# bhansconnect/alphazero-pybind11

Hardware: AMD Instinct MI355X
Metric: self-play games/sec (whole node), Connect4 @ 800 MCTS sims (higher is better)
Workload: dtype bf16

## Files before the change

### alphazero-pybind11_amd/csrc/engine_kernels.h

```cpp
#pragma once
#include <hip/hip_runtime.h>
#include <stdint.h>

#include "dev_games.h"
#include "dev_rng.h"
#include "engine_types.h"

namespace azmi {

constexpr float kNoiseAlphaRatio = 10.83f;

__device__ __forceinline__ uint32_t seat_param(const uint32_t (&a)[4], uint32_t seat) {
  return seat == 0 ? a[0] : seat == 1 ? a[1] : seat == 2 ? a[2] : a[3];
}

__device__ __forceinline__ uint32_t gum_plan(uint32_t m, uint32_t n, uint32_t want, uint32_t& num_c_out, uint32_t& v_per_out) {
  num_c_out = 0; v_per_out = 0;
  if (m <= 1) { if (want == 0) { num_c_out = 1; v_per_out = n; } return 1; }
  uint32_t log2m = 0;
  for (uint32_t v = m - 1; v > 0; v >>= 1) ++log2m;
  if (log2m == 0) log2m = 1;
  const uint32_t d0 = n / (log2m * m);
  const uint32_t base_v = d0 > 1u ? d0 : 1u;
  uint32_t sims_used = 0, num_c = m, count = 0;
// ... 118 lines not shown
  }
  __device__ __forceinline__ size_t tree_base(uint32_t seat) const {
    return (static_cast<size_t>(slot) * P + seat) * ep.cap;
  }
  __device__ __forceinline__ uint32_t tree_id(uint32_t seat) const { return slot * P + seat; }
  __device__ __forceinline__ void raise(uint32_t bit) const {
    if (lane == 0) { atomicOr(&ar.ctl->overflow, bit); ar.ctl->stop = 1; }
  }
  __device__ __forceinline__ void sync_lanes() const { __builtin_amdgcn_fence(__ATOMIC_ACQ_REL, "workgroup"); }
  __device__ __forceinline__ void trace(uint64_t tag) const {
    if (slot != ep.trace_slot || lane != 0) return;
    const uint64_t val = (tag & 0xFF) >= 100 ? wall_clock64() : rng.state;
    if (ar.ctl->rounds < ep.trace_after) return;
    const uint64_t n = ar.trace[0];
    if (n + 1 < ep.trace_cap) { ar.trace[2 * (n + 1)] = tag; ar.trace[2 * (n + 1) + 1] = val; ar.trace[0] = n + 1; }
  }

  __device__ __forceinline__ void load() {
    rng.state = ar.rng[slot];
    coin.state = ar.coin[slot];
    flags = ar.flags[slot];
    const uint64_t w0 = ar.gs_words[0 * ep.S + slot], w1 = ar.gs_words[1 * ep.S + slot],
                   w2 = ar.gs_words[2 * ep.S + slot];
    gs.bb[0] = w0; gs.bb[1] = w1;
    gs.turn = static_cast<uint32_t>(w2); gs.player = static_cast<uint32_t>(w2 >> 32);
#pragma unroll
    for (int p = 0; p < P; ++p) {
      const uint32_t t = slot * P + p;
      t_root[p] = ar.root[t]; t_bump[p] = ar.bump[t]; t_depth[p] = ar.depth[t]; t_tld[p] = ar.tld[t];
    }
    cur = ar.cur[slot]; plen = ar.plen[slot]; ph_rows = ar.ph_count[slot];
    perm = ar.perm[slot];
#pragma unroll
    for (int p = 0; p < P; ++p) {
      const uint32_t* rec = ar.seat_tab + (static_cast<size_t>(perm) * P + p) * kSeatWords;
      sv_w0[p] = rec[0]; sv_w1[p] = rec[1]; sv_eps[p] = __uint_as_float(rec[2]); sv_rt[p] = __uint_as_float(rec[3]);
    }
  }
  __device__ __forceinline__ void store(uint8_t sstate) const {
    if (lane != 0) return;
    ar.rng[slot] = rng.state;
    ar.coin[slot] = coin.state;
    ar.flags[slot] = flags;
    ar.sstate[slot] = sstate;
    ar.gs_words[0 * ep.S + slot] = gs.bb[0];
    ar.gs_words[1 * ep.S + slot] = gs.bb[1];
    ar.gs_words[2 * ep.S + slot] = static_cast<uint64_t>(gs.turn) | (static_cast<uint64_t>(gs.player) << 32);
#pragma unroll
    for (int p = 0; p < P; ++p) {
      const uint32_t t = slot * P + p;
      ar.root[t] = t_root[p]; ar.bump[t] = t_bump[p]; ar.depth[t] = t_depth[p]; ar.tld[t] = t_tld[p];
    }
    ar.cur[slot] = cur; ar.plen[slot] = plen; ar.ph_count[slot] = ph_rows;
  }

  __device__ __forceinline__ void reset_tree(uint32_t seat) {
#pragma unroll
    for (int p = 0; p < P; ++p)
      if (static_cast<uint32_t>(p) == seat) { t_root[p] = 0; t_bump[p] = 1; t_depth[p] = 0; t_tld[p] = 0; }
    const size_t tb = tree_base(seat);
    if (lane == 0) { ar.nodes[tb].n = 0; ar.nodes[tb].q = 0; ar.nodes[tb].pr = 0; ar.nodes[tb].d = 0; ar.nodes[tb].v = 0; ar.nodes[tb].meta = 0; }
    if (ep.gumbel_on) set_gumbel_num_sims(seat, 0);
  }

  enum { kGumTarget = 0, kGumInit = 1, kGumNSurv = 2, kGumPhase = 3, kGumSims = 4, kGumMEff = 5, kGumRemain = 6 };
  __device__ __forceinline__ uint32_t* gum_state(uint32_t seat) const { return ar.gum_state + static_cast<size_t>(tree_id(seat)) * 8; }
  __device__ __forceinline__ float* gum_g(uint32_t seat) const { return ar.gum_g + static_cast<size_t>(tree_id(seat)) * ep.gum_stride; }
  __device__ __forceinline__ uint16_t* gum_surv(uint32_t seat) const { return ar.gum_surv + static_cast<size_t>(tree_id(seat)) * kGumMaxM; }

  __device__ __forceinline__ void reset_gumbel_state(uint32_t seat) const {
    if (lane != 0) return;
    uint32_t* st = gum_state(seat);
    st[kGumInit] = 0; st[kGumNSurv] = 0; st[kGumPhase] = 0; st[kGumSims] = 0; st[kGumMEff] = 0; st[kGumRemain] = 0;
  }
  __device__ __forceinline__ void set_gumbel_num_sims(uint32_t seat, uint32_t n) const {
    if (lane == 0) gum_state(seat)[kGumTarget] = n;
    reset_gumbel_state(seat);
  }
  __device__ __forceinline__ void set_gumbel_target() const {
    if (!ep.gumbel_on) return;
    const uint32_t cp = gs.player;
    const uint32_t target = (flags & kFlagCapped) ? (ep.fast_gumbel ? seat_cap_visits(cp) : 0u) : seat_visits(cp);
    set_gumbel_num_sims(cp, target);
  }
  __device__ __forceinline__ float gumbel01() {
    return 0.0f - 1.0f * az_logf(-az_logf(1.0f - canonical01(rng)));
  }
  __device__ __forceinline__ uint32_t group_max(uint32_t x) const {
    for (int off = 1; off < G; off <<= 1) x = max(x, __shfl_xor(x, off, G));
    return x;
  }
  __device__ __forceinline__ void init_gumbel_state(uint32_t seat, uint32_t k, float p_l) {
    if (k == 0) return;
    uint32_t* st = gum_state(seat);
    const uint32_t target = st[kGumTarget], depth = AZMI_SEL(t_depth, seat);
    const uint32_t remaining = depth < target ? target - depth : 0u;
    if (remaining == 0) return;
    const uint32_t gm = seat_gumbel_m(seat);
    uint32_t m_eff = gm < k ? gm : k;
    m_eff = m_eff < remaining ? m_eff : remaining;
    m_eff = m_eff > 1u ? m_eff : 1u;
    float g_l = 0.0f;
    for (uint32_t i = 0; i < k; ++i) { const float gi = gumbel01(); if (lane == i) g_l = gi; }
    const float score_l = g_l + az_logf(p_l + 1e-20f);
    uint32_t rank_l = 0;
    for (uint32_t j = 0; j < k; ++j) {
// ... 818 lines not shown
              if (b < np) dp[b] = t1;
              if (c < np) dp[c] = t2;
              if (d < np) dp[d] = t3;
            }
            float* dv = ar.h_v + dst0 * (P + 1);
            for (uint32_t e = lane; e < nr * (P + 1); e += G) dv[e] = (e % (P + 1) == term - 1) ? 1.0f : 0.0f;
            for (uint32_t r = lane; r < nr; r += G) {
              const uint32_t* pm = ar.ph_meta + (src0 + sr + r) * 2;
              uint32_t* hm = ar.h_meta + (dst0 + r) * 4;
              hm[0] = slot; hm[1] = game_idx; hm[2] = pm[1]; hm[3] = pm[0];
            }
          }
        }
      } else {
        raise(2u);
      }
    }
    ph_rows = 0;
    if (lane == 0) {
      atomicAdd(&ar.a_scores[static_cast<size_t>(slot) * (P + 1) + (term - 1)], 1.0f);
      if (resigned) atomicAdd(&ar.a_resign[static_cast<size_t>(slot) * (P + 1) + (term - 1)], 1.0f);
      atomicAdd(&ar.a_perm_scores[(static_cast<size_t>(slot) * ep.num_perms + perm) * (P + 1) + (term - 1)], 1.0f);
      atomicAdd(&ar.a_perm_games[static_cast<size_t>(slot) * ep.num_perms + perm], 1u);
      double gd[5]; uint32_t gc[3];
#pragma unroll
      for (int j = 0; j < 5; ++j) gd[j] = ar.g_dsum[j * S + slot];
#pragma unroll
      for (int j = 0; j < 3; ++j) gc[j] = ar.g_cnt[j * S + slot];
      atomicAdd(reinterpret_cast<unsigned long long*>(&ar.a_len[slot]), static_cast<unsigned long long>(gs.turn));
#pragma unroll
      for (int j = 0; j < 5; ++j) { atomicAdd(&ar.a_dsum[j * S + slot], gd[j]); ar.g_dsum[j * S + slot] = 0.0; }
#pragma unroll
      for (int j = 0; j < 3; ++j) { atomicAdd(reinterpret_cast<unsigned long long*>(&ar.a_cnt[j * S + slot]), static_cast<unsigned long long>(gc[j])); ar.g_cnt[j * S + slot] = 0; }
      atomicAdd(&ar.slot_games[slot], 1u);
      const uint32_t pos = atomicAdd(&ar.ctl->ended_count, 1u);
      ar.ended_list[pos] = slot;
    }
  }

  __device__ __forceinline__ void emit_leaf(const typename GM::State& leaf, uint64_t key) const {
    float* row = ar.canon + static_cast<size_t>(slot) * GM::CANON;
    for (uint32_t e = lane; e < static_cast<uint32_t>(GM::CANON); e += G) row[e] = GM::canonical_at(leaf, e);
    if (lane == 0) {
      ar.leaf_key[slot] = key;
      if (ar.leaf_pos) {
        ar.leaf_pos[0 * static_cast<size_t>(ep.S) + slot] = leaf.bb[0];
        ar.leaf_pos[1 * static_cast<size_t>(ep.S) + slot] = leaf.bb[1];
        ar.leaf_pos[2 * static_cast<size_t>(ep.S) + slot] = leaf.player;
      }
    }
  }
  struct NoEarly { __device__ __forceinline__ bool operator()(int, float&, float&) const { return false; } };
  struct NoAfter { __device__ __forceinline__ void operator()(float, float) const {} };
  template <class F = NoPreload, class E = NoEarly, class A = NoAfter>
  __device__ __forceinline__ bool cache_lookup(uint64_t key, uint32_t group, float& hit_pi, float& hit_v, F&& before_loads = F(), E&& early = E(),
                                               A&& after_hit = A()) const {
    uint32_t sh;
    const CacheView cache = ep.num_groups == 1 ? ar.cache : ar.caches[group];
    const int cslot = wave_shard_find<G>(cache, key, lane, &sh, before_loads);
    if (lane == 0) {
      unsigned long long* st = cache.stats + static_cast<size_t>(sh) * 4;
      if (cslot < 0) {
        atomicAdd(&st[1], 1ULL);
      } else {
        atomicAdd(&st[0], 1ULL);
        uint32_t* f = cache.freq + static_cast<size_t>(sh) * kWaveCap + cslot;
        atomicAdd(f, 1u);
        atomicMin(f, 3u);
      }
    }
    static_assert(M <= G, "one lane per policy entry");
    bool have = early(cslot, hit_pi, hit_v);
    if (!have) {
      if (cslot < 0) return false;
      const float* sp = cache.policy + (static_cast<size_t>(sh) * cache.cap + cslot) * M;
      const float* sv = cache.value + (static_cast<size_t>(sh) * cache.cap + cslot) * (P + 1);
      hit_pi = lane < static_cast<uint32_t>(M) ? sp[lane] : 0.0f;
      hit_v = lane <= static_cast<uint32_t>(P) ? sv[lane] : 0.0f;
      after_hit(hit_pi, hit_v);
    }
    if (lane < static_cast<uint32_t>(M)) ar.pi[static_cast<size_t>(slot) * M + lane] = hit_pi;
    if (lane <= static_cast<uint32_t>(P)) ar.v[static_cast<size_t>(slot) * (P + 1) + lane] = hit_v;
    return true;
  }
};

template <class GM, bool kPlayout = false, bool kMover = false>
__device__ __forceinline__ uint32_t round_slot(const EngineParams& ep, const EngineArrays& ar, const uint32_t slot, const uint32_t lane) {
  constexpr int G = GM::GROUP;
  constexpr int P = GM::P;
  if (slot >= ep.S) return 0xFFu;
  if (ar.ctl->stop) return 0xFFu;
  const uint8_t st = ar.sstate[slot];
  if (st == kSlotDone || st == kSlotEnded) { if (ep.cache_on && lane == 0) ar.cache_keys[slot] = 0; return 0xFFu; }
  if constexpr (!kMover) {
    if (st == kSlotQueued) {
      if (lane == 0) {
        const uint32_t group = ar.leaf_group[slot];
        if (ep.cache_on) ar.cache_keys[slot] = cache_key(ar.leaf_key[slot]);
        ar.eval_list[static_cast<size_t>(group) * ep.S + atomicAdd(&ar.ctl->eval_count[group], 1u)] = slot;
        ar.sstate[slot] = kSlotWaitEval;
      }
      return kSlotWaitEval;
    }
  }
  SlotCtx<GM> c(ep, ar, slot, lane);
  c.trace(100);
  c.load();
  if constexpr (kMover) c.flags &= ~kFlagListed;
  c.trace(101);
  uint32_t inline_sims = 0, insert_key_set = 0;
  PathRegs prec;
  bool need_process = (st == kSlotWaitEval);
  if (!need_process) {
    c.start_game();
    c.draw_capped();
    c.set_gumbel_target();
    if (ep.gumbel_on && st == kSlotRestart && !ep.tree_reuse) c.set_gumbel_num_sims(c.gs.player, 0);
  }
  bool have_regs = false;
  float reg_pi = 0.0f, reg_v = 0.0f;
  for (;;) {
    if (need_process) {
      const uint32_t cp = c.gs.player;
      const bool noise = c.seat_eps(cp) > 0 && !(c.flags & kFlagCapped);
      c.process_result(cp, (c.flags & kFlagLeafNeedsNet) != 0, noise, have_regs, reg_pi, reg_v);
      have_regs = false;
      c.trace(102);
      const uint32_t goal = (c.flags & kFlagCapped) ? c.seat_cap_visits(cp) : c.seat_visits(cp);
      if (AZMI_SEL(c.t_depth, cp) >= goal) {
        if (c.make_move(cp)) { if (ep.cache_on && lane == 0) ar.cache_keys[slot] = 0; c.store(kSlotEnded); c.trace(107); return kSlotEnded; }
        c.trace(103);
      }
    }
    const uint32_t cp = c.gs.player;
// ... 310 lines not shown
```

### alphazero-pybind11_amd/csrc/pipe_tree_kernels.h

```cpp
#pragma once
#include "engine_kernels.h"
#include "pipe_types.h"

namespace azmi {

__device__ __forceinline__ unsigned long long g_ld(const unsigned long long* p) { return __hip_atomic_load(p, __ATOMIC_RELAXED, __HIP_MEMORY_SCOPE_AGENT); }
__device__ __forceinline__ uint32_t g_ld(const uint32_t* p) { return __hip_atomic_load(p, __ATOMIC_RELAXED, __HIP_MEMORY_SCOPE_AGENT); }
__device__ __forceinline__ void g_st(unsigned long long* p, unsigned long long v) { __hip_atomic_store(p, v, __ATOMIC_RELAXED, __HIP_MEMORY_SCOPE_AGENT); }
__device__ __forceinline__ void g_st(uint32_t* p, uint32_t v) { __hip_atomic_store(p, v, __ATOMIC_RELAXED, __HIP_MEMORY_SCOPE_AGENT); }


enum : uint32_t { kGrpIdle = 0, kGrpReady = 1, kGrpWait = 2, kGrpPush = 3 };
constexpr uint64_t kFreezeTicks = 200000ull;
__device__ __forceinline__ void pipe_freeze_credit(PipeCtl* pc, uint64_t now, uint64_t& t_last, uint64_t& t_start, bool leader) {
  const uint64_t gap = now - t_last;
  if (gap > kFreezeTicks) {
    t_start += gap;
    if (leader) { atomicAdd(&pc->freezes, 1ull); atomicMax(&pc->freeze_max, static_cast<unsigned long long>(gap)); }
  }
  t_last = now;
}
constexpr uint64_t kMask48 = (1ull << 48) - 1;
constexpr uint32_t kNoSlot = 0xFFFFFFFFu;

// ... 80 lines not shown
    const unsigned long long em = __ballot(on && lane == 0 && res_state == kSlotEnded);
    const unsigned long long dm = __ballot(on && lane == 0 && (res_state == kSlotDone || res_state == 0xFFu));
    const unsigned long long om = __ballot(on && lane == 0);
    const unsigned long long sm = __ballot(on && lane == 0 && was_sim != 0u);
    if (wlane == 0) {
      if (em) atomicAdd(&pe->ended, static_cast<uint32_t>(__popcll(em)));
      if (dm) atomicAdd(&pe->dead, static_cast<uint32_t>(__popcll(dm)));
      if (sm) atomicAdd(&pe->sims, static_cast<unsigned long long>(__popcll(sm)));
      atomicAdd(&pe->moved, static_cast<uint32_t>(__popcll(om)));
    }
  }
  return res_state;
}

#ifndef AZMI_TREE_MINB
#define AZMI_TREE_MINB 2
#endif
template <class GM, int NT, bool PROF, bool TWO = false, bool GUM = false>
__global__ __launch_bounds__(NT, AZMI_TREE_MINB) void k_pipe_tree(PipeKernArgs ka) {
  constexpr int G = GM::GROUP;
  constexpr int P = GM::P;
  static_assert(P == 2 && G == 8 && GM::M == 7, "written for Connect4's 8-lane groups");
  const EngineParams& ep = ka.ep;
  const EngineArrays& ar = ka.ar;
  const PipeArrays& pa = ka.pa;
  const uint32_t wlane = threadIdx.x & 63u, grp = wlane >> 3, lane0 = wlane & 7u;
  uint64_t t_start = wall_clock64(), t_last = t_start;
  PipeCtl* const pc = pa.ctl;
  PipeEpoch* const pe = pa.ep;
  PipeWg* const wc = pa.wg + blockIdx.x;
  const uint32_t rmask = (1u << pa.rshift) - 1u;
  unsigned long long* const myring = pa.rring + (static_cast<size_t>(blockIdx.x) << pa.rshift);
  if (threadIdx.x == 0) {
    unsigned long long t0 = atomicCAS(&pe->t0, 0ull, static_cast<unsigned long long>(t_start));
    if (t0 == 0ull) t0 = t_start;
    atomicMax(&pe->tree_late, static_cast<uint32_t>(t_start > t0 ? t_start - t0 : 0ull));
    const uint32_t before = atomicAdd(&pe->tree_arrived, 1u);
    asm volatile("s_waitcnt vmcnt(0)" :: "v"(before) : "memory");
  }
  __syncthreads();
  if (pa.census_hold != 0u) {
    const unsigned long long t0 = g_ld(&pe->t0);
    if (threadIdx.x == 0 && t_start > t0 && t_start - t0 >= pa.census_hold) atomicAdd(&pe->tree_late_n, 1u);
    while (wall_clock64() < t0 + pa.census_hold) __builtin_amdgcn_s_sleep(32);
    return;
  }
  bool go = g_ld(&ar.ctl->stop) == 0 && g_ld(&pc->err) == 0 && g_ld(&pe->stop) == 0;
  __shared__ uint32_t s_head;
  if (threadIdx.x == 0) s_head = wc->rhead;
  __syncthreads();
  uint64_t pf_pass = 0, pf_idle = 0, pf_n = 0, pf_act = 0, pf_polls = 0, pf_io = 0, pf_lvls = 0, pf_mv = 0;
  uint64_t pf_ph[5] = {0, 0, 0, 0, 0};
  SlotCtx<GM> c(ep, ar, 0u, lane0);

  while (go) {
    const uint64_t pf_t0 = PROF ? wall_clock64() : 0;
    uint32_t lane = lane0;
    asm volatile("" : "+v"(lane));
    c.lane = lane;
    uint32_t my_slot = kNoSlot, tok_seq = 0, tok_move = 0, n_tok = 0, empty_polls = 0, ctl_word = 0;
    uint64_t t_seen = 0;
    bool fresh_pass = true;
    for (;;) {
      const uint32_t h = __builtin_amdgcn_readfirstlane(*const_cast<volatile uint32_t*>(&s_head));
      unsigned long long tok = 0;
      bool here = false;
      if (lane == 0) {
        const uint32_t pos = h + grp;
        tok = g_ld(myring + (pos & rmask));
        here = (tok >> 48) == pipe_lap_tag_r(pos, pa.rshift);
      }
      if ((empty_polls & 3u) == 0u) {
        ctl_word = 0;
        if (wlane == 7) ctl_word = g_ld(&pe->stop) | g_ld(&pc->err) | g_ld(&ar.ctl->stop);
        else if (wlane == 15) ctl_word = g_ld(&pe->sims) >= pa.quota ? 1u : 0u;
        else if (wlane == 23) ctl_word = g_ld(&pe->ended);
        else if (wlane == 31) ctl_word = g_ld(&pe->dead);
      }
      uint32_t stop_seen = __builtin_amdgcn_readlane(ctl_word, 7) | __builtin_amdgcn_readlane(ctl_word, 15);
      {
        const uint32_t w = __builtin_amdgcn_readlane(ctl_word, 23), d = __builtin_amdgcn_readlane(ctl_word, 31);
        const uint32_t with_game = ep.S > d ? ep.S - d : 0u;
        const uint32_t thr = max(1u, static_cast<uint32_t>((static_cast<unsigned long long>(with_game) * pa.idle_num) >> 10));
        if (w >= thr || w + d >= ep.S) stop_seen = 1u;
      }
      const uint64_t now = wall_clock64();
      if (fresh_pass) { t_last = now; fresh_pass = false; }
      else pipe_freeze_credit(pc, now, t_last, t_start, wlane == 0);
      if (now - t_start > pa.soft_ticks) stop_seen = 1u;
      if (now - t_start > pa.cap_ticks) {
        if (wlane == 0) { atomicOr(&pc->err, static_cast<uint32_t>(kPipeErrTimeout)); pc->dbg[16] = __builtin_amdgcn_readlane(ctl_word, 23); pc->dbg[17] = __builtin_amdgcn_readlane(ctl_word, 31); }
        stop_seen = 1u;
      }
      if (stop_seen) {
        if (wlane == 0) g_st(&pe->stop, 1u);
        go = false;
        break;
      }
      if constexpr (PROF) pf_polls += 1;
      const unsigned long long hm = __ballot(here);
      uint32_t k = 0;
      while (k < kTreeWindow && ((hm >> (8 * k)) & 1ull)) ++k;
      if (k == 0u) { ++empty_polls; __builtin_amdgcn_s_sleep(16); continue; }
      if (k < kTreeWindow && pa.take_wait != 0u) {
        if (t_seen == 0) t_seen = now;
        if (now - t_seen <= pa.take_wait) { __builtin_amdgcn_s_sleep(2); continue; }
      }
      uint32_t won = 0;
      if (wlane == 0) won = atomicCAS(&s_head, h, h + k) == h ? 1u : 0u;
      if (__builtin_amdgcn_readfirstlane(won) == 0u) continue;
      n_tok = k;
      {
        const uint32_t sl = static_cast<uint32_t>(__shfl(static_cast<uint32_t>(tok & 0xFFFFull), static_cast<int>(grp * 8), 64));
        const uint32_t sq = static_cast<uint32_t>(__shfl(static_cast<uint32_t>((tok >> 16) & 0xFFFFFFFFull), static_cast<int>(grp * 8), 64));
        if (grp < k) { my_slot = sl & static_cast<uint32_t>(kTokSlotMask); tok_move = (sl >> 15) & 1u; tok_seq = sq; }
      }
      break;
    }
    if (!go) break;
    const uint64_t pf_t1 = PROF ? wall_clock64() : 0;
    if constexpr (PROF) { pf_idle += pf_t1 - pf_t0; pf_n += 1; pf_act += n_tok; }

    if (__ballot(tok_move != 0u) != 0ull) {
      const PipeKernArgs* const kargs = reinterpret_cast<const PipeKernArgs*>(reinterpret_cast<uintptr_t>(__builtin_amdgcn_kernarg_segment_ptr()));
      const uint32_t rs = pipe_move_groups<GM>(kargs->ep, kargs->ar, kargs->pa, tok_move != 0u ? my_slot : kNoSlot);
      asm volatile("s_waitcnt vmcnt(0)" ::: "memory");
      if (tok_move != 0u) { if (rs == kSlotWaitEval) tok_seq = 0u; else my_slot = kNoSlot; }
      if constexpr (PROF) pf_mv += wall_clock64() - pf_t1;
    }

    const uint32_t slot = my_slot != kNoSlot ? my_slot : 0u;
    c.slot = slot;
    uint32_t st = kGrpIdle;
    uint8_t final_state = kSlotWaitEval;
    uint32_t cp = 0, root = 0, goal = 0, seq = 0, mg = 0, gum_active = 0, gum_full = 0;
    bool gum_defer = false;
    size_t tb = 0;
    float fpu_root = 0.0f;
    uint32_t* const path = ar.path + static_cast<size_t>(slot) * ep.max_depth;
    unsigned long long* const res = pa.res + static_cast<size_t>(slot) * kResStride;
    float reg_pi = 0.0f, reg_v = 0.0f;
    uint32_t root_n = 0; float root_v = 0.0f; uint64_t root_meta = 0;
    uint32_t lv_node = 0, lv_n = 0, lv_pp = 0;
    float lv_q = 0.0f, lv_d = 0.0f, lv_v = 0.0f;
    uint64_t lf_meta = 0;
    uint32_t lf_mv = 0, lf_c0 = 0, lf_k = 0, lf_term = 0, lf_player = 0;
    bool fw = false;
    uint32_t fw_node = 0, fw_n = 0, fw_plen = 0;
    float fw_q = 0.0f, fw_d = 0.0f, fw_v = 0.0f;
    uint32_t fl_node = 0xFFFFFFFFu, fl_mv = 0;
    uint64_t fl_meta = 0;
    float fl_pr = 0.0f;
    uint32_t sims_done = 0, sims_mem = 0, l0_hits = 0;
    bool rec_ok = true, answered = false;
    uint64_t cur_key = 0;
    unsigned long long g0 = 0, g1 = 0;
    PendRec pr_in{};
    uint32_t seq_now = 0;
    if (my_slot != kNoSlot) {
      seq_now = g_ld(ar.req_seq + slot);
      if (tok_seq != 0u) {
        while (seq_now != tok_seq) {
          if (wall_clock64() - t_start > pa.cap_ticks) {
            if (lane == 0 && atomicAdd(&pc->dbg[0], 1u) == 0u) { pc->dbg[1] = slot; pc->dbg[2] = tok_seq; pc->dbg[3] = seq_now; pc->dbg[4] = 0xEEEEu; pc->dbg[14] = blockIdx.x; pc->dbg[15] = static_cast<uint32_t>((wall_clock64() - t_start) / 100u); }
            if (lane == 0) atomicOr(&pc->err, static_cast<uint32_t>(kPipeErrTimeout));
            my_slot = kNoSlot;
            break;
          }
          __builtin_amdgcn_s_sleep(2);
          seq_now = g_ld(ar.req_seq + slot);
        }
      }
    }
    __builtin_amdgcn_fence(__ATOMIC_ACQUIRE, "workgroup");
    if (my_slot != kNoSlot) {
      if (tok_seq != 0u) {
        if (lane < static_cast<uint32_t>(GM::M)) g0 = g_ld(res + lane);
        if (lane <= static_cast<uint32_t>(P)) g1 = g_ld(res + kResV + lane);
      }
      pr_in = ar.pend[static_cast<size_t>(slot) * G + lane];
      cur_key = ar.leaf_key[slot];
      c.load();
    }
    const bool on = my_slot != kNoSlot;
    if (on) {
      cp = c.gs.player;
      if constexpr (TWO) mg = c.seat_group(cp) & 1u;
      tb = c.tree_base(cp);
      root = AZMI_SEL(c.t_root, cp);
      goal = (c.flags & kFlagCapped) ? c.seat_cap_visits(cp) : c.seat_visits(cp);
      fpu_root = c.seat_fpu_zero(cp) ? 0.0f : ep.fpu_reduction;
      seq = seq_now;
      rec_ok = (c.flags & kFlagPendRec) != 0;
      st = kGrpReady;
      if constexpr (GUM) {
        if (c.seat_gumbel(cp)) {
          const uint32_t* const gst = c.gum_state(cp);
          gum_active = gst[SlotCtx<GM>::kGumInit];
          gum_defer = gum_active == 0u && gst[SlotCtx<GM>::kGumTarget] > 0u;
          gum_full = c.seat_gumbel_full(cp) ? 1u : 0u;
        }
      }
      { const NodeRec* rr = ar.nodes + tb + root; root_n = rr->n; root_v = rr->v; root_meta = rr->meta; }
      lv_node = pr_in.node; lv_n = pr_in.n; lv_pp = pr_in.pp_mv & 0xFFu;
      lv_q = pr_in.q; lv_d = pr_in.d; lv_v = pr_in.v;
      lf_meta = pr_in.leaf_meta;
      lf_mv = pr_in.pp_mv >> 8;
      lf_c0 = meta_ch0(lf_meta); lf_k = meta_nch(lf_meta); lf_term = meta_term(lf_meta); lf_player = meta_player(lf_meta);
      if (c.flags & kFlagReqOut) {
        for (uint32_t spins = 0;; ++spins) {
          if (spins != 0u || tok_seq == 0u) {
            if (lane < static_cast<uint32_t>(GM::M)) g0 = g_ld(res + lane);
            if (lane <= static_cast<uint32_t>(P)) g1 = g_ld(res + kResV + lane);
          }
          const bool ok = (lane >= static_cast<uint32_t>(GM::M) || static_cast<uint32_t>(g0 >> 32) == seq) &&
                          (lane > static_cast<uint32_t>(P) || static_cast<uint32_t>(g1 >> 32) == seq);
          if (c.group_all(ok)) break;
          if (wall_clock64() - t_start > pa.cap_ticks) {
            if (lane == 0 && atomicAdd(&pc->dbg[0], 1u) == 0u) { pc->dbg[1] = slot; pc->dbg[2] = seq; pc->dbg[3] = c.flags; pc->dbg[4] = static_cast<uint32_t>(g1 >> 32); pc->dbg[5] = static_cast<uint32_t>(g0 >> 32); }
            if (lane == 0) atomicOr(&pc->err, static_cast<uint32_t>(kPipeErrTimeout));
            st = kGrpIdle;
            break;
          }
          __builtin_amdgcn_s_sleep(2);
        }
        if (st == kGrpReady) {
          reg_pi = lane < static_cast<uint32_t>(GM::M) ? __uint_as_float(static_cast<uint32_t>(g0)) : 0.0f;
          reg_v = lane <= static_cast<uint32_t>(P) ? __uint_as_float(static_cast<uint32_t>(g1)) : 0.0f;
          if (lane < static_cast<uint32_t>(GM::M)) ar.pi[static_cast<size_t>(slot) * GM::M + lane] = reg_pi;
          if (lane <= static_cast<uint32_t>(P)) ar.v[static_cast<size_t>(slot) * (P + 1) + lane] = reg_v;
          c.flags &= ~kFlagReqOut;
          answered = true;
        }
      } else if (c.flags & kFlagLeafNeedsNet) {
        if (lane < static_cast<uint32_t>(GM::M)) reg_pi = ar.pi[static_cast<size_t>(slot) * GM::M + lane];
        if (lane <= static_cast<uint32_t>(P)) reg_v = ar.v[static_cast<size_t>(slot) * (P + 1) + lane];
      }
    }
    if (ep.cache_on) {
      const unsigned long long am = __ballot(answered && lane == 0);
      if (am) {
        uint32_t base = 0;
        if (wlane == 0) base = atomicAdd(&pe->ins_count, static_cast<uint32_t>(__popcll(am)));
        base = __builtin_amdgcn_readfirstlane(base);
        if (answered) {
          const uint32_t idx = base + static_cast<uint32_t>(__popcll(am & ((1ull << (grp * 8)) - 1ull)));
          if (idx < pa.ins_cap) {
            if (lane == 0) pa.ins_key[idx] = cur_key;
            if constexpr (TWO) { if (lane == 1 && pa.ins_grp) pa.ins_grp[idx] = static_cast<uint8_t>(mg); }
            if (lane < static_cast<uint32_t>(GM::M)) pa.ins_pi[static_cast<size_t>(idx) * GM::M + lane] = reg_pi;
            if (lane <= static_cast<uint32_t>(P)) pa.ins_v[static_cast<size_t>(idx) * (P + 1) + lane] = reg_v;
          } else if (lane == 0) {
            g_st(&pe->stop, 1u);
          }
        }
      }
    }
    const uint64_t pf_t2 = PROF ? wall_clock64() : 0;
    if constexpr (PROF) pf_io += pf_t2 - pf_t1;

    bool listed = false;
    if (st == kGrpReady) {
      uint32_t inline_sims = 0;
      float cpuct = ep.cpuct, fpu_red = ep.fpu_reduction;
      asm volatile("" : "+s"(cpuct), "+s"(fpu_red));
      for (;;) {
        if (AZMI_SEL(c.t_depth, cp) + 1 >= goal || c.cur == root || (GUM && gum_defer)) {
          c.flags |= kFlagListed;
          listed = true;
          st = kGrpIdle;
          break;
        }
        const uint64_t ph0 = PROF ? wall_clock64() : 0;
        if (!rec_ok) {
          const bool from_net = (c.flags & kFlagLeafNeedsNet) != 0;
          c.template process_result<true>(cp, from_net, false, from_net, reg_pi, reg_v);
          root_n += 1;
          sims_mem += 1;
          fw = false; fl_node = 0xFFFFFFFFu;
        } else {
          const bool from_net = (c.flags & kFlagLeafNeedsNet) != 0;
          float val[P + 1];
          if (lf_term != 0) {
#pragma unroll
            for (int i = 0; i <= P; ++i) val[i] = (static_cast<int>(lf_term) - 1 == i) ? 1.0f : 0.0f;
          } else {
            float p = 0.0f;
            if (from_net) {
              val[0] = c.template bcast_lane<0>(reg_v); val[1] = c.template bcast_lane<1>(reg_v); val[2] = c.template bcast_lane<2>(reg_v);
              p = c.bcast(reg_pi, static_cast<int>(lf_mv));
              if (lane >= lf_k) p = 0.0f;
            } else {
#pragma unroll
              for (int i = 0; i <= P; ++i) val[i] = static_cast<float>(1.0 / (P + 1));
              const float ksum = static_cast<float>(lf_k & 0xFFu);
              if (lane < lf_k) p = (ksum == 0.0f) ? 0.0f : 1.0f / ksum;
            }
            const float sum = c.seqsum8(lane < lf_k ? p : 0.0f);
            p = p / sum;
            if (lane < lf_k) ar.nodes[tb + lf_c0 + lane].pr = p;
            fl_pr = p;
          }
          fl_node = c.cur; fl_mv = lf_mv; fl_meta = lf_meta;
          const float draw_share = val[P] / static_cast<int32_t>(P);
          const uint32_t plen = c.plen;
          float nq = 0.0f, nd = 0.0f, nv = lv_v;
          if (lane < plen) {
            const float vv = ((lv_pp == 0) ? val[0] : val[1]) + draw_share;
            nq = (lv_q * static_cast<float>(lv_n) + vv) / static_cast<float>(lv_n + 1);
            nd = (lv_d * static_cast<float>(lv_n) + val[P]) / static_cast<float>(lv_n + 1);
            NodeRec* nr = ar.nodes + tb + lv_node;
            nr->q = nq; nr->d = nd;
            if (lv_n == 0) { nv = ((lf_player == 0) ? val[0] : val[1]) + draw_share; nr->v = nv; }
            nr->n = lv_n + 1;
          }
          fw_node = lv_node; fw_n = lv_n + 1; fw_q = nq; fw_d = nd; fw_v = nv; fw_plen = plen; fw = true;
          root_n += 1;
          if (lane == 0) ar.nodes[tb + root].n = root_n;
#pragma unroll
          for (int p = 0; p < P; ++p) if (static_cast<uint32_t>(p) == cp) c.t_depth[p] += 1;
          sims_done += 1;
        }
        const uint64_t ph1 = PROF ? wall_clock64() : 0;
        typename GM::State leaf = c.gs;
        uint32_t cur = root, plen = 0, n = root_n;
        uint64_t meta = root_meta;
        float v_cur = root_v;
        bool prefix = true, failed = false;
        while (n > 0 && meta_term(meta) == 0) {
          if (plen >= ep.max_depth) { failed = true; break; }
          if (lane == 0) path[plen] = cur;
          uint32_t k = meta_nch(meta); const uint32_t c0 = meta_ch0(meta);
          if (k == 0) { failed = true; break; }
          const uint32_t t_node = c.bcast(fw_node, static_cast<int>(plen & 7u));
          const bool in_regs = cur == fl_node;
          const NodeRec* const cr = ar.nodes + tb + c0 + (lane < k ? lane : k - 1u);
          uint32_t n_l = cr->n; float q_l = cr->q, p_l = cr->pr, d_l = cr->d, v_l = cr->v; uint64_t m_l = cr->meta;
          float sqrt_n = SlotCtx<GM>::select_parent(n);
          asm volatile("" : "+v"(sqrt_n), "+v"(k));
          {
            const bool have = lane < k, mem = have && !in_regs;
            n_l = mem ? n_l : 0u; q_l = mem ? q_l : 0.0f; d_l = mem ? d_l : 0.0f; v_l = mem ? v_l : 0.0f;
            p_l = mem ? p_l : have ? fl_pr : 0.0f;
            m_l = mem ? m_l : have ? meta_pack(0, 0, fl_mv, 0, 0) : 0ull;
          }
          if (!in_regs) {
            if (fw && prefix && plen < fw_plen && plen < 8u) {
              const uint32_t t_n = c.bcast(fw_n, static_cast<int>(plen));
              const float t_q = c.bcast(fw_q, static_cast<int>(plen)), t_d = c.bcast(fw_d, static_cast<int>(plen)), t_v = c.bcast(fw_v, static_cast<int>(plen));
              if (c0 + lane == t_node) { n_l = t_n; q_l = t_q; d_l = t_d; v_l = t_v; if (t_node == fl_node) m_l = fl_meta; }
            }
          }
          const float fpu = (cur == root) ? fpu_root : fpu_red;
          uint32_t best;
          if constexpr (GUM) {
            if (gum_active != 0u && cur == root) best = c.gumbel_next_root_child(cp, k, n_l, q_l, p_l);
            else if (gum_active != 0u && gum_full != 0u) best = c.gumbel_interior_select(cp, k, n_l, q_l, p_l, v_cur);
            else best = c.select_among(k, n_l, q_l, p_l, v_cur, sqrt_n, cpuct, fpu);
          } else {
            best = c.select_among(k, n_l, q_l, p_l, v_cur, sqrt_n, cpuct, fpu);
          }
          const uint32_t nxt = c0 + best;
          const uint32_t s_n = c.bcast(n_l, static_cast<int>(best));
          const float s_q = c.bcast(q_l, static_cast<int>(best)), s_d = c.bcast(d_l, static_cast<int>(best)), s_v = c.bcast(v_l, static_cast<int>(best));
          const uint64_t s_m = c.bcast(m_l, static_cast<int>(best));
          if (plen < 8u) {
            if (lane == plen) { lv_node = nxt; lv_n = s_n; lv_q = s_q; lv_d = s_d; lv_v = s_v; lv_pp = meta_player(meta); }
            prefix = prefix && plen < fw_plen && nxt == t_node;
          } else {
            prefix = false;
          }
          cur = nxt; n = s_n; meta = s_m; v_cur = s_v;
          GM::play(leaf, meta_mv(meta));
          ++plen;
        }
        if (failed) { c.raise(8u); final_state = kSlotDone; st = kGrpIdle; break; }
        const uint64_t ph2 = PROF ? wall_clock64() : 0;
        if constexpr (PROF) pf_lvls += plen;
        c.cur = cur; c.plen = plen;
        rec_ok = plen <= 8u;
#pragma unroll
        for (int p = 0; p < P; ++p) if (static_cast<uint32_t>(p) == cp) c.t_tld[p] += plen;
        uint32_t term = meta_term(meta);
        lf_k = meta_nch(meta); lf_c0 = meta_ch0(meta); lf_mv = 0; lf_meta = meta;
        if (n == 0) {
          term = GM::terminal(leaf);
          const uint64_t keep = meta_pack(0, 0, meta_mv(meta), leaf.player, term);
          if (!c.template expand_node<true>(cp, cur, leaf, keep, lf_c0, lf_k, &lf_mv)) { final_state = kSlotDone; st = kGrpIdle; break; }
          lf_meta = meta_pack(lf_c0, lf_k, meta_mv(meta), leaf.player, term);
        }
        lf_term = term; lf_player = leaf.player;
        const uint64_t ph3 = PROF ? wall_clock64() : 0;
        const bool needs_net = term == 0 && !c.seat_eval_random(cp);
        c.flags = needs_net ? (c.flags | kFlagLeafNeedsNet) : (c.flags & ~kFlagLeafNeedsNet);
        if (needs_net) {
          const uint64_t key = GM::key(leaf);
          unsigned long long l0a = 0, l0b = 0;
          const uint64_t lkey = TWO ? key ^ (mg ? kPipeGroupSalt : 0ull) : key;
          const unsigned long long* const le = pa.l0 + static_cast<size_t>(pipe_l0_entry(lkey, pa.l0_mask)) * kResStride;
          const bool hit = ep.cache_on && c.cache_lookup(key, mg, reg_pi, reg_v,
            [&]() {
              if (pa.l0) {
                if (lane < static_cast<uint32_t>(GM::M)) l0a = g_ld(le + lane);
                if (lane <= static_cast<uint32_t>(P)) l0b = g_ld(le + kResV + lane);
              }
            },
            [&](int cslot, float& o_pi, float& o_v) -> bool {
              if (!pa.l0) return false;
              const bool okl = (lane >= static_cast<uint32_t>(GM::M) || static_cast<uint32_t>(l0a >> 32) == pipe_l0_tag(lkey, lane)) &&
                               (lane > static_cast<uint32_t>(P) || static_cast<uint32_t>(l0b >> 32) == pipe_l0_tag(lkey, kResV + lane));
              if (!c.group_all(okl)) return false;
              o_pi = lane < static_cast<uint32_t>(GM::M) ? __uint_as_float(static_cast<uint32_t>(l0a)) : 0.0f;
              o_v = lane <= static_cast<uint32_t>(P) ? __uint_as_float(static_cast<uint32_t>(l0b)) : 0.0f;
              if (cslot < 0) l0_hits += 1;
              return true;
            },
            [&](float h_pi, float h_v) {
              if (pa.l0 && pa.l0_wb) {
                unsigned long long* const we = pa.l0 + static_cast<size_t>(pipe_l0_entry(lkey, pa.l0_mask)) * kResStride;
                if (lane < static_cast<uint32_t>(GM::M)) g_st(we + lane, (static_cast<unsigned long long>(pipe_l0_tag(lkey, lane)) << 32) | __float_as_uint(h_pi));
                if (lane <= static_cast<uint32_t>(P)) g_st(we + kResV + lane, (static_cast<unsigned long long>(pipe_l0_tag(lkey, kResV + lane)) << 32) | __float_as_uint(h_v));
              }
            });
          if (!hit) {
            cur_key = key;
            seq = seq + 1u == 0u ? 1u : seq + 1u;
            uint32_t pos = 0;
            if (lane == 0) pos = atomicAdd(TWO ? pipe_tail_of(pc, mg) : &pc->tail, 1u);
            pos = c.template bcast_lane<0>(pos);
            const uint64_t payload = lane == 0 ? leaf.bb[0] : lane == 1 ? leaf.bb[1] : lane == 2 ? (static_cast<uint64_t>(slot) | (static_cast<uint64_t>(leaf.player) << 16))
                                                                                                  : static_cast<uint64_t>(seq);
            const unsigned long long rtag = (pa.test_drop != 0u && pos == pa.test_drop) ? pipe_lap_tag(pos + kPipeRing) : pipe_lap_tag(pos);
            if (lane < kReqGranules)
              g_st((TWO ? pipe_ring_of(pa, mg) : pa.ring) + static_cast<size_t>(pos & (kPipeRing - 1u)) * kReqGranules + lane, (rtag << 48) | (payload & kMask48));
            if (lane < 3u) ar.leaf_pos[static_cast<size_t>(lane) * ep.S + slot] = lane == 2u ? static_cast<uint64_t>(leaf.player) : payload;
            if constexpr (TWO) { if (lane == 3u) ar.leaf_group[slot] = static_cast<uint8_t>(mg); }
            st = kGrpPush;
          }
        }
        if constexpr (PROF) {
          const uint64_t ph4 = wall_clock64();
          pf_ph[0] += ph1 - ph0; pf_ph[1] += ph2 - ph1; pf_ph[2] += ph3 - ph2; pf_ph[3] += ph4 - ph3; pf_ph[4] += 1;
        }
        if (st == kGrpPush) break;
        if (++inline_sims >= pa.max_inline) break;
        if (static_cast<uint32_t>(__popcll(__ballot(lane == 0))) < pa.min_active) break;
      }
    }
    const uint64_t pf_t3 = PROF ? wall_clock64() : 0;
    if constexpr (PROF) pf_pass += pf_t3 - pf_t2;


    if (on) {
      if (st == kGrpPush) c.flags |= kFlagReqOut;
      if (lane == 0) {
        if (sims_done) ar.c_sims[slot] += sims_done;
        if (st == kGrpPush) { ar.c_evals[slot] += 1; ar.leaf_key[slot] = cur_key; }
      }
      if (rec_ok) {
        PathRegs r;
        r.node = lv_node; r.n = lv_n; r.q = lv_q; r.d = lv_d; r.v = lv_v; r.pp = lv_pp; r.mv = lf_mv; r.leaf_meta = lf_meta;
        c.store_pend(r);
        c.flags |= kFlagPendRec;
      } else {
        c.flags &= ~kFlagPendRec;
      }
      c.store(final_state);
    }
    {
      const bool tok_out = on && lane == 0 && (st == kGrpReady || listed);
      const unsigned long long rm = __ballot(tok_out);
      uint32_t base = 0;
      if (rm && wlane == 0) base = atomicAdd(&wc->rtail, static_cast<uint32_t>(__popcll(rm)));
      asm volatile("s_waitcnt vmcnt(0)" ::: "memory");
      if (on && lane == 0) g_st(ar.req_seq + slot, seq);
      if (rm) {
        base = __builtin_amdgcn_readfirstlane(base);
        if (tok_out) {
          const uint32_t pos = base + static_cast<uint32_t>(__popcll(rm & ((1ull << (grp * 8)) - 1ull)));
          g_st(myring + (pos & rmask), (pipe_lap_tag_r(pos, pa.rshift) << 48) | static_cast<unsigned long long>(slot) | (listed ? kTokMove : 0ull));
        }
      }
    }
    {
      uint32_t x = lane == 0 ? sims_done + sims_mem : 0u;
#pragma unroll
      for (int off = 32; off > 0; off >>= 1) x += __shfl_xor(x, off, 64);
      if (wlane == 0 && x) atomicAdd(&pe->sims, static_cast<unsigned long long>(x));
      if (pa.l0) {
        uint32_t y = lane == 0 ? l0_hits : 0u;
#pragma unroll
        for (int off = 32; off > 0; off >>= 1) y += __shfl_xor(y, off, 64);
        if (wlane == 0 && y) atomicAdd(&pc->l0_hits, static_cast<unsigned long long>(y));
      }
      const unsigned long long fm = __ballot(on && lane == 0 && final_state == kSlotDone);
      if (wlane == 0 && fm) atomicAdd(&pe->dead, static_cast<uint32_t>(__popcll(fm)));
    }
    if constexpr (PROF) pf_io += wall_clock64() - pf_t3;
  }

  if (wlane == 0) g_st(&pe->stop, 1u);
  if (PROF && wlane == 0) {
    atomicAdd(&pc->prof[0], pf_pass); atomicAdd(&pc->prof[1], pf_idle); atomicAdd(&pc->prof[2], pf_n); atomicAdd(&pc->prof[3], pf_act);
    atomicAdd(&pc->prof[4], pf_polls); atomicAdd(&pc->prof[5], pf_io);
    atomicAdd(&pc->prof[9], pf_ph[0]); atomicAdd(&pc->prof[10], pf_ph[1]); atomicAdd(&pc->prof[11], pf_ph[2]); atomicAdd(&pc->prof[12], pf_ph[3]);
    atomicAdd(&pc->prof[13], pf_ph[4]); atomicAdd(&pc->prof[14], pf_lvls); atomicAdd(&pc->prof[15], pf_mv); atomicAdd(&pc->prof[6], static_cast<unsigned long long>(wall_clock64() - t_start));
  }
  asm volatile("s_waitcnt vmcnt(0)" ::: "memory");
  __syncthreads();
  if (threadIdx.x == 0) { wc->rhead = s_head; atomicAdd(&pe->tree_done, 1u); }
}

template <class GM, int NT, bool DIAG = false>
__global__ __launch_bounds__(NT, 2) void k_pipe_tree_generic(PipeKernArgs ka) {
  constexpr int P = GM::P;
  const EngineParams& ep = ka.ep;
  const EngineArrays& ar = ka.ar;
  const PipeArrays& pa = ka.pa;
  const uint32_t wlane = threadIdx.x & 63u, grp = wlane >> 3, lane = wlane & 7u;
  uint64_t t_start = wall_clock64(), t_last = t_start;
  PipeCtl* const pc = pa.ctl;
  PipeEpoch* const pe = pa.ep;
  PipeWg* const wc = pa.wg + blockIdx.x;
  uint32_t* const phase_word = &wc->pad[2 + (threadIdx.x >> 6)];
  const bool diag_on = DIAG && g_ld(&pc->err) == 0u;
#define AZMI_GEN_PHASE(x) do { if (DIAG && wlane == 0 && diag_on) g_st(phase_word, static_cast<uint32_t>(x) | (static_cast<uint32_t>((wall_clock64() - t_start) / 1000u) << 8)); } while (0)
  AZMI_GEN_PHASE(1);
  if (DIAG && wlane == 0 && diag_on) g_st(&wc->pad[6 + (threadIdx.x >> 6)], static_cast<uint32_t>(t_start));
  const uint32_t rmask = (1u << pa.rshift) - 1u;
  unsigned long long* const myring = pa.rring + (static_cast<size_t>(blockIdx.x) << pa.rshift);
  if (threadIdx.x == 0) {
    unsigned long long t0 = atomicCAS(&pe->t0, 0ull, static_cast<unsigned long long>(t_start));
    if (t0 == 0ull) t0 = t_start;
    atomicMax(&pe->tree_late, static_cast<uint32_t>(t_start > t0 ? t_start - t0 : 0ull));
    const uint32_t before = atomicAdd(&pe->tree_arrived, 1u);
    asm volatile("s_waitcnt vmcnt(0)" :: "v"(before) : "memory");
  }
  __syncthreads();
  AZMI_GEN_PHASE(2);
  if (pa.census_hold != 0u) {
    const unsigned long long t0 = g_ld(&pe->t0);
    if (threadIdx.x == 0 && t_start > t0 && t_start - t0 >= pa.census_hold) atomicAdd(&pe->tree_late_n, 1u);
    while (wall_clock64() < t0 + pa.census_hold) __builtin_amdgcn_s_sleep(32);
    return;
  }
  bool go = g_ld(&ar.ctl->stop) == 0 && g_ld(&pc->err) == 0 && g_ld(&pe->stop) == 0;
  __shared__ uint32_t s_head;
  if (threadIdx.x == 0) s_head = wc->rhead;
  __syncthreads();
  const PipeKernArgs* const kargs = reinterpret_cast<const PipeKernArgs*>(reinterpret_cast<uintptr_t>(__builtin_amdgcn_kernarg_segment_ptr()));
  uint64_t seg_max[3] = {0, 0, 0}, sg_prev = DIAG ? __builtin_amdgcn_s_memtime() : 0ull;
  uint64_t ph_max[5] = {0, 0, 0, 0, 0};
  uint64_t gap_rt = 0, gap_sq = 0, sq_last = DIAG ? __builtin_amdgcn_s_memtime() : 0ull;
// ... 172 lines not shown
```

Measured before the change: 6737.

## Defer and trim global stores in pipelined tree pass

Adds a slimmer per-pass slot state store that skips unchanged fields (coin, game state, root, ph_count). Path entries, root visit counts and pi/v rows are now kept in registers and written once at the end of the pass instead of on every step. Cache stat atomics are merged into one, the redundant pi/v writes on cache hits are dropped, and l0 hit counts are accumulated per wave and flushed once at kernel exit. The aim is less global store and atomic traffic. The risk is correctness if any skipped field is in fact modified during a pass, or if the deferred writes are missing on some path.

Result: faster. 6813, median of 6 (+1.1%).

```diff
diff --git a/alphazero-pybind11_amd/csrc/engine_kernels.h b/alphazero-pybind11_amd/csrc/engine_kernels.h
--- a/alphazero-pybind11_amd/csrc/engine_kernels.h
+++ b/alphazero-pybind11_amd/csrc/engine_kernels.h
@@ -194,6 +194,18 @@
       ar.root[t] = t_root[p]; ar.bump[t] = t_bump[p]; ar.depth[t] = t_depth[p]; ar.tld[t] = t_tld[p];
     }
     ar.cur[slot] = cur; ar.plen[slot] = plen; ar.ph_count[slot] = ph_rows;
+  }
+  __device__ __forceinline__ void store_pass(uint8_t sstate) const {
+    if (lane != 0) return;
+    ar.rng[slot] = rng.state;
+    ar.flags[slot] = flags;
+    ar.sstate[slot] = sstate;
+#pragma unroll
+    for (int p = 0; p < P; ++p) {
+      const uint32_t t = slot * P + p;
+      ar.bump[t] = t_bump[p]; ar.depth[t] = t_depth[p]; ar.tld[t] = t_tld[p];
+    }
+    ar.cur[slot] = cur; ar.plen[slot] = plen;
   }
 
   __device__ __forceinline__ void reset_tree(uint32_t seat) {
@@ -1118,7 +1130,7 @@
   }
   struct NoEarly { __device__ __forceinline__ bool operator()(int, float&, float&) const { return false; } };
   struct NoAfter { __device__ __forceinline__ void operator()(float, float) const {} };
-  template <class F = NoPreload, class E = NoEarly, class A = NoAfter>
+  template <bool PASS = false, class F = NoPreload, class E = NoEarly, class A = NoAfter>
   __device__ __forceinline__ bool cache_lookup(uint64_t key, uint32_t group, float& hit_pi, float& hit_v, F&& before_loads = F(), E&& early = E(),
                                                A&& after_hit = A()) const {
     uint32_t sh;
@@ -1126,10 +1138,11 @@
     const int cslot = wave_shard_find<G>(cache, key, lane, &sh, before_loads);
     if (lane == 0) {
       unsigned long long* st = cache.stats + static_cast<size_t>(sh) * 4;
+      if constexpr (PASS) atomicAdd(&st[cslot < 0 ? 1 : 0], 1ULL);
       if (cslot < 0) {
-        atomicAdd(&st[1], 1ULL);
+        if constexpr (!PASS) atomicAdd(&st[1], 1ULL);
       } else {
-        atomicAdd(&st[0], 1ULL);
+        if constexpr (!PASS) atomicAdd(&st[0], 1ULL);
         uint32_t* f = cache.freq + static_cast<size_t>(sh) * kWaveCap + cslot;
         atomicAdd(f, 1u);
         atomicMin(f, 3u);
@@ -1145,8 +1158,10 @@
       hit_v = lane <= static_cast<uint32_t>(P) ? sv[lane] : 0.0f;
       after_hit(hit_pi, hit_v);
     }
-    if (lane < static_cast<uint32_t>(M)) ar.pi[static_cast<size_t>(slot) * M + lane] = hit_pi;
-    if (lane <= static_cast<uint32_t>(P)) ar.v[static_cast<size_t>(slot) * (P + 1) + lane] = hit_v;
+    if constexpr (!PASS) {
+      if (lane < static_cast<uint32_t>(M)) ar.pi[static_cast<size_t>(slot) * M + lane] = hit_pi;
+      if (lane <= static_cast<uint32_t>(P)) ar.v[static_cast<size_t>(slot) * (P + 1) + lane] = hit_v;
+    }
     return true;
   }
 };
diff --git a/alphazero-pybind11_amd/csrc/pipe_tree_kernels.h b/alphazero-pybind11_amd/csrc/pipe_tree_kernels.h
--- a/alphazero-pybind11_amd/csrc/pipe_tree_kernels.h
+++ b/alphazero-pybind11_amd/csrc/pipe_tree_kernels.h
@@ -156,6 +156,7 @@
   uint64_t pf_pass = 0, pf_idle = 0, pf_n = 0, pf_act = 0, pf_polls = 0, pf_io = 0, pf_lvls = 0, pf_mv = 0;
   uint64_t pf_ph[5] = {0, 0, 0, 0, 0};
   SlotCtx<GM> c(ep, ar, 0u, lane0);
+  uint32_t wave_l0_hits = 0;
 
   while (go) {
     const uint64_t pf_t0 = PROF ? wall_clock64() : 0;
@@ -257,10 +258,15 @@
     float fl_pr = 0.0f;
     uint32_t sims_done = 0, sims_mem = 0, l0_hits = 0;
     bool rec_ok = true, answered = false;
+    bool path_held = false, rows_held = false;
     uint64_t cur_key = 0;
     unsigned long long g0 = 0, g1 = 0;
     PendRec pr_in{};
     uint32_t seq_now = 0;
+    auto store_path_image = [&]() {
+      const uint32_t up = SlotCtx<GM>::template dpp_u<0x111>(lv_node);
+      if (lane < min(c.plen, 8u)) path[lane] = lane == 0 ? root : up;
+    };
     if (my_slot != kNoSlot) {
       seq_now = g_ld(ar.req_seq + slot);
       if (tok_seq != 0u) {
@@ -331,8 +337,7 @@
         if (st == kGrpReady) {
           reg_pi = lane < static_cast<uint32_t>(GM::M) ? __uint_as_float(static_cast<uint32_t>(g0)) : 0.0f;
           reg_v = lane <= static_cast<uint32_t>(P) ? __uint_as_float(static_cast<uint32_t>(g1)) : 0.0f;
-          if (lane < static_cast<uint32_t>(GM::M)) ar.pi[static_cast<size_t>(slot) * GM::M + lane] = reg_pi;
-          if (lane <= static_cast<uint32_t>(P)) ar.v[static_cast<size_t>(slot) * (P + 1) + lane] = reg_v;
+          rows_held = true;
           c.flags &= ~kFlagReqOut;
           answered = true;
         }
@@ -378,6 +383,7 @@
         const uint64_t ph0 = PROF ? wall_clock64() : 0;
         if (!rec_ok) {
           const bool from_net = (c.flags & kFlagLeafNeedsNet) != 0;
+          if (lane == 0) ar.nodes[tb + root].n = root_n;
           c.template process_result<true>(cp, from_net, false, from_net, reg_pi, reg_v);
           root_n += 1;
           sims_mem += 1;
@@ -420,7 +426,6 @@
           }
           fw_node = lv_node; fw_n = lv_n + 1; fw_q = nq; fw_d = nd; fw_v = nv; fw_plen = plen; fw = true;
           root_n += 1;
-          if (lane == 0) ar.nodes[tb + root].n = root_n;
 #pragma unroll
           for (int p = 0; p < P; ++p) if (static_cast<uint32_t>(p) == cp) c.t_depth[p] += 1;
           sims_done += 1;
@@ -433,7 +438,7 @@
         bool prefix = true, failed = false;
         while (n > 0 && meta_term(meta) == 0) {
           if (plen >= ep.max_depth) { failed = true; break; }
-          if (lane == 0) path[plen] = cur;
+          if (plen >= 8u && lane == 0) path[plen] = cur;
           uint32_t k = meta_nch(meta); const uint32_t c0 = meta_ch0(meta);
           if (k == 0) { failed = true; break; }
           const uint32_t t_node = c.bcast(fw_node, static_cast<int>(plen & 7u));
@@ -483,6 +488,7 @@
         if constexpr (PROF) pf_lvls += plen;
         c.cur = cur; c.plen = plen;
         rec_ok = plen <= 8u;
+        if (rec_ok) path_held = true; else { store_path_image(); path_held = false; }
 #pragma unroll
         for (int p = 0; p < P; ++p) if (static_cast<uint32_t>(p) == cp) c.t_tld[p] += plen;
         uint32_t term = meta_term(meta);
@@ -502,7 +508,7 @@
           unsigned long long l0a = 0, l0b = 0;
           const uint64_t lkey = TWO ? key ^ (mg ? kPipeGroupSalt : 0ull) : key;
           const unsigned long long* const le = pa.l0 + static_cast<size_t>(pipe_l0_entry(lkey, pa.l0_mask)) * kResStride;
-          const bool hit = ep.cache_on && c.cache_lookup(key, mg, reg_pi, reg_v,
+          const bool hit = ep.cache_on && c.template cache_lookup<true>(key, mg, reg_pi, reg_v,
             [&]() {
               if (pa.l0) {
                 if (lane < static_cast<uint32_t>(GM::M)) l0a = g_ld(le + lane);
@@ -526,6 +532,7 @@
                 if (lane <= static_cast<uint32_t>(P)) g_st(we + kResV + lane, (static_cast<unsigned long long>(pipe_l0_tag(lkey, kResV + lane)) << 32) | __float_as_uint(h_v));
               }
             });
+          if (hit) rows_held = true;
           if (!hit) {
             cur_key = key;
             seq = seq + 1u == 0u ? 1u : seq + 1u;
@@ -557,8 +564,13 @@
 
     if (on) {
       if (st == kGrpPush) c.flags |= kFlagReqOut;
+      if (path_held) store_path_image();
+      if (rows_held && (c.flags & kFlagLeafNeedsNet) && st != kGrpPush) {
+        if (lane < static_cast<uint32_t>(GM::M)) ar.pi[static_cast<size_t>(slot) * GM::M + lane] = reg_pi;
+        if (lane <= static_cast<uint32_t>(P)) ar.v[static_cast<size_t>(slot) * (P + 1) + lane] = reg_v;
+      }
       if (lane == 0) {
-        if (sims_done) ar.c_sims[slot] += sims_done;
+        if (sims_done) { ar.c_sims[slot] += sims_done; ar.nodes[tb + root].n = root_n; }
         if (st == kGrpPush) { ar.c_evals[slot] += 1; ar.leaf_key[slot] = cur_key; }
       }
       if (rec_ok) {
@@ -569,7 +581,7 @@
       } else {
         c.flags &= ~kFlagPendRec;
       }
-      c.store(final_state);
+      c.store_pass(final_state);
     }
     {
       const bool tok_out = on && lane == 0 && (st == kGrpReady || listed);
@@ -589,13 +601,13 @@
     {
       uint32_t x = lane == 0 ? sims_done + sims_mem : 0u;
 #pragma unroll
-      for (int off = 32; off > 0; off >>= 1) x += __shfl_xor(x, off, 64);
+      for (int off = 32; off >= 8; off >>= 1) x += __shfl_xor(x, off, 64);
       if (wlane == 0 && x) atomicAdd(&pe->sims, static_cast<unsigned long long>(x));
       if (pa.l0) {
         uint32_t y = lane == 0 ? l0_hits : 0u;
 #pragma unroll
-        for (int off = 32; off > 0; off >>= 1) y += __shfl_xor(y, off, 64);
-        if (wlane == 0 && y) atomicAdd(&pc->l0_hits, static_cast<unsigned long long>(y));
+        for (int off = 32; off >= 8; off >>= 1) y += __shfl_xor(y, off, 64);
+        wave_l0_hits += __builtin_amdgcn_readfirstlane(y);
       }
       const unsigned long long fm = __ballot(on && lane == 0 && final_state == kSlotDone);
       if (wlane == 0 && fm) atomicAdd(&pe->dead, static_cast<uint32_t>(__popcll(fm)));
@@ -603,6 +615,7 @@
     if constexpr (PROF) pf_io += wall_clock64() - pf_t3;
   }
 
+  if (wlane == 0 && wave_l0_hits) atomicAdd(&pc->l0_hits, static_cast<unsigned long long>(wave_l0_hits));
   if (wlane == 0) g_st(&pe->stop, 1u);
   if (PROF && wlane == 0) {
     atomicAdd(&pc->prof[0], pf_pass); atomicAdd(&pc->prof[1], pf_idle); atomicAdd(&pc->prof[2], pf_n); atomicAdd(&pc->prof[3], pf_act);
```
